# nv-tlabs/NKSR

Hardware: AMD Instinct MI355X
Metric: reconstructed points/sec (solve+mesh) (higher is better)
Workload: dtype f32

## Files before the change

### include/nksr_hip.h

```cpp
#ifndef NKSR_HIP_H
#define NKSR_HIP_H
#include <stddef.h>
#include <stdint.h>

#ifdef __cplusplus
extern "C" {
#endif

#define NKSR_MAX_DEPTH 6
#define NKSR_OK 0
#define NKSR_ERR_ARG (-1)
#define NKSR_ERR_HIP (-2)
#define NKSR_ERR_CAPACITY (-3)

const char* nksr_last_error(void);
int nksr_version(void);

typedef struct {
    int32_t n;
    int32_t offset;
    const int64_t* keys;
    const int32_t* ijk;
    const int32_t* nbr;
    const int64_t* hkeys;
// ... 98 lines not shown
    const int32_t* row_index;
    int64_t level_base;
} nksr_siteset_t;

int nksr_assemble_count(const nksr_hier_t* h, void* workspace, int32_t* rowcount, int32_t* crosscount, int32_t* samelow,
                        int32_t* indeg, void* stream);
size_t nksr_assemble_workspace_bytes(const nksr_hier_t* h);
size_t nksr_assemble_split_bytes(const nksr_hier_t* h, int64_t total_rows);
int nksr_assemble(const nksr_hier_t* h, const nksr_siteset_t* sets, int nsets, float reg, int col_bits,
                  void* workspace, const int32_t* rowptr, const int32_t* indeg, const int32_t* samelow,
                  const int32_t* mir_off, int col_format, int32_t* cols_out, float* vals_out, float* diag_out,
                  uint64_t* mir_keys, float* mir_vals, float* b_out, void* split_scratch, size_t split_scratch_bytes, void* stream);
int nksr_place_mirrors(const uint64_t* keys_sorted, const float* vals_sorted, int64_t n, int col_bits,
                       const int32_t* rowptr, const int32_t* mirptr, int col_format, int32_t* cols_out, float* vals_out,
                       void* stream);

size_t nksr_spmv_workspace_bytes(int64_t nnz);
int nksr_spmv_plan(const int32_t* rowptr, int32_t M, int64_t nnz, int col_format, void* workspace, void* stream);
int nksr_spmv_csr(const int32_t* rowptr, const void* cols, const float* vals, int32_t M, int64_t nnz, int col_format,
                  const float* x, float* y, void* workspace, void* stream);
int nksr_pack_cols21(const int32_t* cols32, int64_t n_padded, uint64_t* packed_out, void* stream);
int nksr_spmv_set_variant(int v);
size_t nksr_pcg_workspace_bytes(int32_t M, int64_t nnz);
struct nksr_coarse_precond_s;
int nksr_pcg_solve(const int32_t* rowptr, const void* cols, const float* vals, const float* diag, int32_t M,
                   int64_t nnz, int col_format, const float* b, float* x, float tol, int max_iter, int check_every,
                   void* workspace, const struct nksr_coarse_precond_s* coarse_precond, double* info_out, void* stream);
int nksr_pcg_profile(int enable, double* ms_out, int64_t* launches_out);
int64_t nksr_pcg_profile_samples(float* ms_out, int64_t capacity);
int nksr_pcg_profile_bytes(double* algorithmic_out, double* physical_out);
// ... 283 lines not shown
```

### nksr_amd/csrc/assemble.hip

```cpp
#include "common.h"
#include <stdlib.h>

#define ASM_WAVES 1

struct AsmArgs {
    nksr_hier_t hier;
    nksr_siteset_t sets[3];
    int nsets;
    int M;
    int col_bits;
    float reg;
    float* blocks[NKSR_MAX_DEPTH];
    float* bvec[NKSR_MAX_DEPTH];
    int32_t* nsites[NKSR_MAX_DEPTH];
    int32_t* colmap[NKSR_MAX_DEPTH];
    int col_format;
};

__device__ __forceinline__ int row_level(const nksr_hier_t& h, int row) {
    int d = 0;
    while (d + 1 < h.depth && row >= h.lv[d + 1].offset) ++d;
    return d;
}

// ... 7 lines not shown
    const uint32_t t = kk / 192u, m = kk - t * 192u;
    return (int64_t)(t * 192u + 3u * (m & 63u) + (m >> 6));
}

typedef float asm_f32x16 __attribute__((ext_vector_type(16)));

__device__ __forceinline__ float asm_row_value(const nksr_siteset_t& S, int64_t q, int L, int d, int col) {
    if (!S.level_stride) return S.val[(q * L + d) * 27 + col];
    const int dd = col / 27, s = col - dd * 27;
    const int64_t site = S.ncomp == 1 ? q : q / 3;
    const int64_t row = (S.row_index ? (int64_t)S.row_index[site] : site * S.ncomp) + (q - site * S.ncomp);
    return S.val[((int64_t)(d + dd - S.level_base) * S.level_stride + row) * 27 + s];
}

template <int NT>
__device__ __forceinline__ void cell_blocks_finalize(const AsmArgs& A, int d, int c, int lane, asm_f32x16 (&acc)[NT], int total) {
    const nksr_level_t& lv = A.hier.lv[d];
    const int T = (A.hier.depth - d) * 27;
    const int j = lane & 31, half = lane >> 5;
    if (lane == 0) A.nsites[d][c] = total;
    if (total == 0) return;
    float* out = A.blocks[d] + (int64_t)c * 27 * T;
    float* bv = A.bvec[d] + (int64_t)c * 27;
    const int nb = (lane < 27) ? lv.nbr[(int64_t)c * 27 + lane] : -1;
    const unsigned long long need = __ballot(nb >= 0);
#pragma unroll
    for (int n = 0; n < NT; ++n) {
        const int col = 32 * n + j;
#pragma unroll
        for (int r = 0; r < 16; ++r) {
            const int s = (r & 3) + 8 * (r >> 2) + 4 * half;
            if (s < 27 && ((need >> s) & 1ull)) {
                if (col < T) out[s * T + col] = acc[n][r];
                else if (col == T) bv[s] = acc[n][r];
            }
        }
    }
}

#define ASM_PART_ROWS 128
#define ASM_TRIP 4
__host__ __device__ __forceinline__ int asm_level_parts(int d) {
    const int k = d >= 2 ? (1 << (2 * (d - 2))) : 1;
    return k > 64 ? 64 : k;
}
__device__ __forceinline__ int asm_cell_rows(const AsmArgs& A, int d, int c) {
    int R = 0;
    for (int si = 0; si < A.nsets; ++si) R += (A.sets[si].end[d][c] - A.sets[si].start[d][c]) * A.sets[si].ncomp;
    return R;
// ... 27 lines not shown
__device__ __forceinline__ void asm_lm_mfma(const AsmLanePtr<NT>& P, int r0, int r_hi, int half, int j, float w, float (&b)[ASM_TRIP][NT], asm_f32x16 (&acc)[NT]) {
#pragma unroll
    for (int u = 0; u < ASM_TRIP; ++u) {
        const bool ok = r0 + 2 * u + half < r_hi;
        float v[NT];
#pragma unroll
        for (int n = 0; n < NT; ++n) v[n] = (ok && P.on[n]) ? b[u][n] : 0.f;
        const float a = (j < 27) ? w * v[0] : 0.f;
#pragma unroll
        for (int n = 0; n < NT; ++n) acc[n] = __builtin_amdgcn_mfma_f32_32x32x2f32(a, v[n], acc[n], 0, 0, 0);
    }
}
template <int NT>
__device__ __forceinline__ void asm_lm_pointers(const AsmArgs& A, int d, int lane, AsmLanePtr<NT>& P) {
    const nksr_siteset_t& S = A.sets[0];
    const int L = A.hier.depth;
    const int T = (L - d) * 27;
    const int j = lane & 31;
#pragma unroll
    for (int n = 0; n < NT; ++n) {
        const int col = 32 * n + j;
        const int dd = col / 27, sl = col - dd * 27;
        P.on[n] = col < T || (col == T && S.target);
        P.mul[n] = (col == T && S.target) ? 1 : 27;
        P.p[n] = (col == T && S.target) ? S.target : S.val + (col < T ? (int64_t)(d + dd - S.level_base) * S.level_stride * 27 + sl : (int64_t)(d - S.level_base) * S.level_stride * 27);
    }
}
template <int NT>
__device__ __forceinline__ void asm_accumulate_lm(const AsmArgs& A, int d, int r_lo, int r_hi, int lane, asm_f32x16 (&acc)[NT]) {
    if (r_hi <= r_lo) return;
    const nksr_siteset_t& S = A.sets[0];
    const int j = lane & 31, half = lane >> 5;
    AsmLanePtr<NT> P;
    asm_lm_pointers<NT>(A, d, lane, P);
    const float w = S.weight;
    float bA[ASM_TRIP][NT], bB[ASM_TRIP][NT];
    asm_lm_load<NT>(P, r_lo, r_lo, r_hi, half, bA);
    for (int r0 = r_lo; r0 < r_hi; r0 += 4 * ASM_TRIP) {
        const int r1 = r0 + 2 * ASM_TRIP, r2 = r0 + 4 * ASM_TRIP;
        if (r1 < r_hi) asm_lm_load<NT>(P, r1, r_lo, r_hi, half, bB);
// ... 75 lines not shown
    if (c >= A.hier.lv[d].n) return;
    asm_f32x16 acc[NT];
#pragma unroll
    for (int n = 0; n < NT; ++n)
#pragma unroll
        for (int r = 0; r < 16; ++r) acc[n][r] = 0.f;
    for (int p = 0; p < nsplit; ++p) {
        const float* in = scratch + ((int64_t)c * nsplit + p) * (NT * 16 * 64) + lane;
#pragma unroll
        for (int n = 0; n < NT; ++n)
#pragma unroll
            for (int r = 0; r < 16; ++r) acc[n][r] += in[(n * 16 + r) * 64];
    }
    int total = 0;
    for (int si = 0; si < A.nsets; ++si) total += A.sets[si].end[d][c] - A.sets[si].start[d][c];
    cell_blocks_finalize<NT>(A, d, c, lane, acc, total);
}

template <int NT>
__global__ void __launch_bounds__(ASM_WAVES * 64) k_cell_blocks_seq(AsmArgs A, int d, int nsplit) {
    const int wave = threadIdx.x >> 6, lane = threadIdx.x & 63;
    const int c = blockIdx.x * ASM_WAVES + wave;
    if (c >= A.hier.lv[d].n) return;
    asm_f32x16 tot[NT];
#pragma unroll
    for (int n = 0; n < NT; ++n)
#pragma unroll
        for (int r = 0; r < 16; ++r) tot[n][r] = 0.f;
    const int R = asm_cell_rows(A, d, c);
    for (int p = 0; p < nsplit; ++p) {
        int lo, hi;
// ... 2 lines not shown
#pragma unroll
        for (int n = 0; n < NT; ++n)
#pragma unroll
            for (int r = 0; r < 16; ++r) acc[n][r] = 0.f;
        if (hi > lo) {
            if (asm_is_row_list(A)) asm_accumulate_lm<NT>(A, d, A.sets[0].start[d][c] + lo, A.sets[0].start[d][c] + hi, lane, acc);
            else asm_accumulate_rows<NT>(A, d, c, lo, hi, lane, acc);
        }
#pragma unroll
        for (int n = 0; n < NT; ++n)
#pragma unroll
            for (int r = 0; r < 16; ++r) tot[n][r] += acc[n][r];
    }
    int total = 0;
    for (int si = 0; si < A.nsets; ++si) total += A.sets[si].end[d][c] - A.sets[si].start[d][c];
    cell_blocks_finalize<NT>(A, d, c, lane, tot, total);
}

template <int NT, bool LM>
__global__ void __launch_bounds__(ASM_WAVES * 64) k_cell_blocks(AsmArgs A, int d) {
    const int wave = threadIdx.x >> 6, lane = threadIdx.x & 63;
    const nksr_level_t& lv = A.hier.lv[d];
    const int c = blockIdx.x * ASM_WAVES + wave;
    if (c >= lv.n) return;
    const int L = A.hier.depth;
    const int T = (L - d) * 27;
    const int j = lane & 31, half = lane >> 5;
    asm_f32x16 acc[NT];
#pragma unroll
    for (int n = 0; n < NT; ++n)
#pragma unroll
        for (int r = 0; r < 16; ++r) acc[n][r] = 0.f;
    int total = 0;
    if (LM && asm_is_row_list(A)) {
        const int k0 = A.sets[0].start[d][c], k1 = A.sets[0].end[d][c];
        total = k1 > k0 ? k1 - k0 : 0;
        asm_accumulate_lm<NT>(A, d, k0, k1, lane, acc);
        cell_blocks_finalize<NT>(A, d, c, lane, acc, total);
        return;
    }
    for (int si = 0; si < A.nsets; ++si) {
        const nksr_siteset_t& S = A.sets[si];
        const int k0 = S.start[d][c], k1 = S.end[d][c];
        if (k0 >= k1) continue;
        total += k1 - k0;
        const int64_t q0 = (int64_t)k0 * S.ncomp;
        const int nrows = (k1 - k0) * S.ncomp;
        const float w = S.weight;
        if (!LM) {
            for (int m0 = 0; m0 < nrows; m0 += 2) {
                const bool valid = m0 + half < nrows;
                const int64_t q = q0 + m0 + half;
                const float* ra = S.val + (q * L + d) * 27;
// ... 143 lines not shown

template <int NQ> struct cols_u { float v[NQ]; } __attribute__((packed, aligned(4)));
template <int NQ>
__device__ __forceinline__ void load_cols(const float* __restrict__ row, int lane, int T, float out[NQ]) {
    const int t0 = NQ * lane;
    if (t0 + NQ <= T) {
        const cols_u<NQ> c = *reinterpret_cast<const cols_u<NQ>*>(row + t0);
#pragma unroll
        for (int q = 0; q < NQ; ++q) out[q] = c.v[q];
    } else {
#pragma unroll
        for (int q = 0; q < NQ; ++q) out[q] = (t0 + q < T) ? row[t0 + q] : 0.f;
    }
}

template <int NQ>
__global__ void __launch_bounds__(ASM_WAVES * 64) k_row_fill(AsmArgs A, const int32_t* __restrict__ rowptr,
                                                             const int32_t* __restrict__ indeg, const int32_t* __restrict__ samelow,
                                                             const int32_t* __restrict__ mir_off,
                                                             int32_t* __restrict__ cols_out, float* __restrict__ vals_out,
                                                             float* __restrict__ diag_out, uint64_t* __restrict__ mir_keys,
                                                             float* __restrict__ mir_vals,
                                                             float* __restrict__ b_out, int row_begin, int row_end) {
    extern __shared__ __attribute__((aligned(16))) float lds[];
    const int wave = threadIdx.x >> 6, lane = threadIdx.x & 63;
    const int row = row_begin + blockIdx.x * ASM_WAVES + wave;
    if (row >= row_end) return;
    const nksr_hier_t& h = A.hier;
    const int L = h.depth;
    const int d = row_level(h, row);
    const nksr_level_t& lv = h.lv[d];
    const int i = row - lv.offset;
    const int ix = lv.ijk[i * 3], iy = lv.ijk[i * 3 + 1], iz = lv.ijk[i * 3 + 2];
    const int nslots = (L - d) * 125;
    const int T = (L - d) * 27;
    float* acc = lds + wave * (NKSR_MAX_DEPTH * 125);
    for (int t = lane; t < nslots; t += 64) acc[t] = 0.f;

    const int cme = (lane < 27) ? lv.nbr[(int64_t)i * 27 + lane] : -1;
    const int nse = (cme >= 0) ? A.nsites[d][cme] : 0;
    unsigned long long act = __ballot(nse > 0);
    float bl = (nse > 0) ? A.bvec[d][(int64_t)cme * 27 + (26 - lane)] : 0.f;
#pragma unroll
    for (int o = 32; o > 0; o >>= 1) bl += __shfl_xor(bl, o);
    if (lane == 0) b_out[row] = bl;

    int edd[NQ], esx[NQ], esy[NQ], esz[NQ];
#pragma unroll
    for (int q = 0; q < NQ; ++q) {
        const int t = NQ * lane + q, s = t % 27;
        edd[q] = t / 27;
        esx[q] = s / 9 - 1; esy[q] = (s / 3) % 3 - 1; esz[q] = s % 3 - 1;
    }
    constexpr int RF_BATCH = 4;
    float vb[2][RF_BATCH][NQ];
    int sp[2][RF_BATCH];
    auto fetch = [&](int buf) {
#pragma unroll
        for (int u = 0; u < RF_BATCH; ++u) {
            sp[buf][u] = -1;
// ... 21 lines not shown
                    acc[dd * 125 + (rz * 5 + ry) * 5 + rx] += vb[buf][u][q];
                }
            }
        }
    };
    fetch(0);
    while (sp[0][0] >= 0) {
        fetch(1);
        accumulate(0);
        if (sp[1][0] < 0) break;
        fetch(0);
        accumulate(1);
    }

    const int32_t* cm = A.colmap[d] + (int64_t)i * nslots;
    int64_t lpos = (int64_t)rowptr[row] + indeg[row];
    int64_t opos = lpos + samelow[row];
    int64_t mpos = (int64_t)mir_off[row];
    for (int t0 = 0; t0 < nslots; t0 += 64) {
        const int t = t0 + lane;
        const int cv = (t < nslots) ? cm[t] : -1;
        const bool up = cv >= 0, low = cv <= -2, mir = up && t >= 125;
        const unsigned long long mu = __ballot(up), ml = __ballot(low), mm = __ballot(mir);
        const unsigned long long below = (1ull << lane) - 1ull;
        if (up | low) {
            const float v = acc[t];
            const int64_t k = up ? opos + __popcll(mu & below) : lpos + __popcll(ml & below);
            const int64_t ph = csr_phys(k, A.col_format);
            cols_out[ph] = up ? cv : -2 - cv;
            vals_out[ph] = v;
// ... 17 lines not shown
}

__global__ void k_place_mirrors(const uint64_t* __restrict__ keys, const float* __restrict__ vals, int64_t n, int col_bits,
                                const int32_t* __restrict__ rowptr, const int32_t* __restrict__ mirptr,
                                int32_t* __restrict__ cols_out, float* __restrict__ vals_out, int fmt) {
    int64_t m = (int64_t)blockIdx.x * blockDim.x + threadIdx.x;
    if (m >= n) return;
    const uint64_t key = keys[m];
    const int r = (int)(key & (((uint64_t)1 << col_bits) - 1));
    const int src = (int)(key >> col_bits);
    const int64_t ph = csr_phys((int64_t)rowptr[r] + (m - (int64_t)mirptr[r]), fmt);
    cols_out[ph] = src;
    vals_out[ph] = vals[m];
}

static int fill_args(AsmArgs& A, const nksr_hier_t* h, const nksr_siteset_t* sets, int nsets, float reg, int col_bits,
                     void* workspace) {
    if (h->depth < 1 || h->depth > NKSR_MAX_DEPTH) return nksr_set_error(NKSR_ERR_ARG, "bad depth %d", h->depth);
    if (nsets < 0 || nsets > 3) return nksr_set_error(NKSR_ERR_ARG, "at most 3 site sets");
    memset(&A, 0, sizeof(A));
    A.hier = *h;
    for (int s = 0; s < nsets; ++s) {
        if (!(sets[s].weight >= 0.f)) return nksr_set_error(NKSR_ERR_ARG, "site-set weights must be >= 0 (set %d: %g)", s, (double)sets[s].weight);
        A.sets[s] = sets[s];
    }
    A.nsets = nsets;
    A.M = h->lv[h->depth - 1].offset + h->lv[h->depth - 1].n;
    A.col_bits = col_bits;
    A.reg = reg;
    if (col_bits < 1 || col_bits > 32 || ((int64_t)1 << col_bits) < A.M) return nksr_set_error(NKSR_ERR_ARG, "col_bits too small");
// ... 36 lines not shown
extern "C" int nksr_assemble_count(const nksr_hier_t* h, void* workspace, int32_t* rowcount, int32_t* crosscount, int32_t* samelow,
                                   int32_t* indeg, void* stream) {
    AsmArgs A;
    int M = h->lv[h->depth - 1].offset + h->lv[h->depth - 1].n;
    int cb = 1;
    while (((int64_t)1 << cb) < M) ++cb;
    int rc = fill_args(A, h, nullptr, 0, 0.f, cb, workspace);
    if (rc) return rc;
    if (A.M <= 0) return NKSR_OK;
    hipLaunchKernelGGL(k_row_count, dim3(nksr_blocks(A.M, ASM_WAVES * RC_RUN)), dim3(ASM_WAVES * 64), 0, (hipStream_t)stream, A, rowcount,
                       crosscount, samelow, indeg);
    NKSR_CHECK_LAUNCH();
    return NKSR_OK;
}

extern "C" int nksr_assemble(const nksr_hier_t* h, const nksr_siteset_t* sets, int nsets, float reg, int col_bits,
                             void* workspace, const int32_t* rowptr, const int32_t* indeg, const int32_t* samelow,
                             const int32_t* mir_off, int col_format,
                             int32_t* cols_out, float* vals_out, float* diag_out, uint64_t* mir_keys, float* mir_vals,
                             float* b_out, void* split_scratch, size_t split_scratch_bytes, void* stream) {
    AsmArgs A;
    int rc = fill_args(A, h, sets, nsets, reg, col_bits, workspace);
    if (rc) return rc;
    if (col_format < 0 || col_format > 2) return nksr_set_error(NKSR_ERR_ARG, "col_format must be 0, 1 or 2");
    A.col_format = col_format;
    if (A.M <= 0) return NKSR_OK;
    hipStream_t st = (hipStream_t)stream;
    const dim3 blk(ASM_WAVES * 64);
    const size_t lds = (size_t)ASM_WAVES * NKSR_MAX_DEPTH * 125 * sizeof(float);
    int64_t total_rows = 0;
    bool lm = false;
    for (int si = 0; si < nsets; ++si) {
        total_rows += sets[si].n * sets[si].ncomp;
        if (si > 0 && (sets[si].level_stride != 0) != lm) return nksr_set_error(NKSR_ERR_ARG, "site sets mix site-major and level-major rows");
        if (sets[si].level_base < 0 || sets[si].level_base >= h->depth || (sets[si].level_base > 0 && !sets[si].level_stride))
            return nksr_set_error(NKSR_ERR_ARG, "site set: level_base needs level-major rows and a level of the hierarchy");
        lm = sets[si].level_stride != 0;
        for (int d = 0; d < sets[si].level_base; ++d)
            if (h->lv[d].n > 0) return nksr_set_error(NKSR_ERR_ARG, "site set: rows start at level %d but level %d of the hierarchy has cells", (int)sets[si].level_base, d);
    }
    for (int d = 0; d < h->depth; ++d) {
        const int n = h->lv[d].n;
        if (n <= 0) continue;
        const int T = (h->depth - d) * 27, NT = (T + 32) / 32;
// ... 14 lines not shown
                case 5: CELLSPLIT(5); break;
                default: CELLSPLIT(6); break;
            }
        } else {
            switch (NT) {
                case 1: if (lm) hipLaunchKernelGGL((k_cell_blocks<1, true>), grid, blk, 0, st, A, d); else hipLaunchKernelGGL((k_cell_blocks<1, false>), grid, blk, 0, st, A, d); break;
                case 2: if (lm) hipLaunchKernelGGL((k_cell_blocks<2, true>), grid, blk, 0, st, A, d); else hipLaunchKernelGGL((k_cell_blocks<2, false>), grid, blk, 0, st, A, d); break;
                case 3: if (lm) hipLaunchKernelGGL((k_cell_blocks<3, true>), grid, blk, 0, st, A, d); else hipLaunchKernelGGL((k_cell_blocks<3, false>), grid, blk, 0, st, A, d); break;
                case 4: if (lm) hipLaunchKernelGGL((k_cell_blocks<4, true>), grid, blk, 0, st, A, d); else hipLaunchKernelGGL((k_cell_blocks<4, false>), grid, blk, 0, st, A, d); break;
                case 5: if (lm) hipLaunchKernelGGL((k_cell_blocks<5, true>), grid, blk, 0, st, A, d); else hipLaunchKernelGGL((k_cell_blocks<5, false>), grid, blk, 0, st, A, d); break;
                default: if (lm) hipLaunchKernelGGL((k_cell_blocks<6, true>), grid, blk, 0, st, A, d); else hipLaunchKernelGGL((k_cell_blocks<6, false>), grid, blk, 0, st, A, d); break;
            }
        }
        NKSR_CHECK_LAUNCH();
    }
    for (int d = 0; d < h->depth; ++d) {
        const int n = h->lv[d].n;
        if (n <= 0) continue;
        const int T = (h->depth - d) * 27;
        const int r0 = h->lv[d].offset, r1 = r0 + n;
        const dim3 grid(nksr_blocks(n, ASM_WAVES));
#define ROWFILL(NQ) hipLaunchKernelGGL((k_row_fill<NQ>), grid, blk, lds, st, A, rowptr, indeg, samelow, mir_off, cols_out, vals_out, diag_out, \
                                       mir_keys, mir_vals, b_out, r0, r1)
        if (T > 128) ROWFILL(3); else if (T > 64) ROWFILL(2); else ROWFILL(1);
        NKSR_CHECK_LAUNCH();
    }
    return NKSR_OK;
}

extern "C" int nksr_place_mirrors(const uint64_t* keys_sorted, const float* vals_sorted, int64_t n, int col_bits,
                                  const int32_t* rowptr, const int32_t* mirptr, int col_format, int32_t* cols_out, float* vals_out,
                                  void* stream) {
    if (n <= 0) return NKSR_OK;
    if (col_format < 0 || col_format > 2) return nksr_set_error(NKSR_ERR_ARG, "col_format must be 0, 1 or 2");
    hipLaunchKernelGGL(k_place_mirrors, dim3(nksr_blocks(n, 256)), dim3(256), 0, (hipStream_t)stream, keys_sorted, vals_sorted, n,
                       col_bits, rowptr, mirptr, cols_out, vals_out, col_format);
    NKSR_CHECK_LAUNCH();
    return NKSR_OK;
}
```

### nksr_amd/fields/assembly.py

```python
import ctypes as C
import time

import torch

from .. import _lib, ops
from .._lib import SiteSetT, call, ptr, stream
from ._timing import _tick


def _sets_from_operator(fld, fused_op, coarse_from, sets, keep):
    first, last = fused_op['span'][0], fused_op['span'][1]
    st_all, en_all = first.clamp(min=0), (last + 1).contiguous()
    off = fld.svh.offsets
    S = sets[0]
    S.n, S.ncomp, S.weight = fused_op['rows_total'], 1, 1.0
    if fused_op.get('row_format') == 'factors':
        dense = fld._dense_coarse_rows(fused_op, int(coarse_from))
        S.val, S.level_base = ptr(dense), int(coarse_from)
        keep.append(dense)
    else:
        S.val = ptr(fused_op['rows_all'])
    S.level_stride = fused_op['rows_total']
    for d in range(fld.svh.depth):
        nd = fld.svh.level(d).num_voxels
# ... 74 lines not shown
    del ws
    ks, vs = ops.sort_pairs(mir_k, mir_v.view(torch.int32), end_bit=col_bits)
    del mir_k, mir_v
    call('nksr_place_mirrors', ptr(ks), ptr(vs.view(torch.float32)), n_mir, col_bits, ptr(rowptr), ptr(mirptr), fmt, ptr(cols),
         ptr(vals), stream())
    del ks, vs
    td = _tick('asm:mirrors', td)
    if fmt == 1:
        packed = torch.empty(npad // 3, dtype=torch.int64, device=dev)
        call('nksr_pack_cols21', ptr(cols), npad, ptr(packed), stream())
        cols = packed
    if coarse_from is None:
        fld.nnz = nnz
    del keep
    return rowptr, cols, vals, diag, b
```

### nksr_amd/fields/coarse_precond.py

```python
import ctypes as C
import os
import time

import torch

from .. import ops
from .._lib import PC_MAX_STEPS, CoarsePrecondT, call, ptr, stream
from ._timing import _tick

PC_RATIO = 40.0
PC_DROP_TOL = 0.005


def _pack_block(rowptr, cols, vals, diag, n, row_seg, counts, drop):
    dev = rowptr.device
    ar = torch.arange(n, dtype=torch.int64, device=dev)
    old_of_new = torch.argsort(row_seg.long() * n + ar)
    new_of_old = torch.empty_like(old_of_new)
    new_of_old[old_of_new] = ar
    seg_base = torch.cat([counts.new_zeros(1), torch.cumsum(counts, 0)]).to(torch.int32)
    row_seg_new = row_seg[old_of_new].contiguous()
    o2n, n2o = old_of_new.to(torch.int32), new_of_old.to(torch.int32)
    lens = torch.empty(n + 1, dtype=torch.int32, device=dev)
    lens[n:] = 0
    call('nksr_coarse_pack_count', ptr(rowptr), ptr(cols), ptr(vals), ptr(diag), n, ptr(o2n), drop, ptr(lens), stream())
    prow = ops.exclusive_sum_i32(lens)
    kept = int(prow[n].item())
    packed = torch.empty(max(kept, 1), dtype=torch.int32, device=dev)
    dis = torch.empty(n, dtype=torch.float32, device=dev)
    call('nksr_coarse_pack', ptr(rowptr), ptr(cols), ptr(vals), ptr(diag), n, ptr(o2n), ptr(n2o), ptr(row_seg_new), ptr(seg_base), ptr(prow),
         drop, ptr(packed), ptr(dis), stream())
    return packed, prow, dis, o2n, seg_base, row_seg_new, kept


def coarse_precond(fld, op, reg_weight, segments=None, sites=None, override=None):
    cfg = fld.solver_config.get('coarse_precond')
    L = fld.svh.depth
    if cfg is False:
        return None
    cfg = dict(cfg) if isinstance(cfg, dict) else dict(override or {})
    for k, e in (('first_level', 'NKSR_PC_LEVEL'), ('steps', 'NKSR_PC_STEPS'), ('ratio', 'NKSR_PC_RATIO')):
        if e in os.environ and k not in cfg:
            cfg[k] = float(os.environ[e])
    c0 = int(cfg.get('first_level', 2))
    off = fld.svh.offsets
    M = fld.svh.num_unknowns
    if not 0 < c0 < L or M - off[c0] < 1:
        return None
    n = M - off[c0]
    nseg = segments.nseg if segments is not None else 1
    td = _tick('_', time.perf_counter())
    if op is not None:
        rowptr, cols, vals, diag, _ = fld.assemble(None, None, None, 1.0, 1.0, reg_weight, coarse_from=c0, fused_op=op)
    else:
        rowptr, cols, vals, diag, _ = fld.assemble(reg_weight=reg_weight, coarse_from=c0, **sites)
    td = _tick('pc:assemble', td)
    lam = torch.empty(nseg, dtype=torch.float32, device=fld.device)
    coef = torch.empty(nseg * (1 + 2 * PC_MAX_STEPS), dtype=torch.float32, device=fld.device)
    row_seg = segments.unknown_seg[off[c0]:].contiguous() if segments is not None else None
    pc = CoarsePrecondT()
    pc.first, pc.n, pc.steps, pc.lambda_scale, pc.ratio = off[c0], n, int(cfg.get('steps', 8)), float(cfg.get('lambda_scale', 1.1)), float(cfg.get('ratio', PC_RATIO))
    gersh = torch.empty(nseg, dtype=torch.float32, device=fld.device)
    pc.lambda_, pc.coef = ptr(lam), ptr(coef)
    nnz = int(cols.numel())
    info = {'first_level': c0, 'unknowns': n, 'nnz': nnz, 'steps': int(pc.steps), 'lambda': lam}
    rs = row_seg if row_seg is not None else torch.zeros(n, dtype=torch.int32, device=fld.device)
    counts = torch.bincount(rs.long(), minlength=nseg)
    if cfg.get('packed', os.environ.get('NKSR_PC_PACKED', '1') != '0') and int(counts.max()) < 65536:
        drop = float(cfg.get('drop', os.environ.get('NKSR_PC_DROP', PC_DROP_TOL)))
        packed, prow, dis, o2n, seg_base, row_seg_new, kept = _pack_block(rowptr, cols, vals, diag, n, rs, counts, drop)
        info.update(nnz_kept=kept + n, drop=drop)
        work = torch.empty(4 * n, dtype=torch.float32, device=fld.device)
        if 'steps' not in cfg and (segments is not None or n >= 100000):
            pc.steps = 10
            info['steps'] = 10
        pc.format, pc.row_seg, pc.work = 1, ptr(row_seg_new), ptr(work)
        pc.packed, pc.packed_rowptr, pc.dis, pc.old_of_new, pc.seg_base = ptr(packed), ptr(prow), ptr(dis), ptr(o2n), ptr(seg_base)
        call('nksr_coarse_lambda_max_packed', C.byref(pc), nseg, 8, ptr(work), ptr(lam), stream())
        call('nksr_coarse_gershgorin', C.byref(pc), nseg, ptr(work), ptr(gersh), stream())
        pc.gersh = ptr(gersh)
        info.update(packed=True, gershgorin=gersh, keep=(packed, prow, dis, o2n, seg_base, row_seg_new, work, lam, coef, gersh))
        td = _tick('pc:pack+lambda', td)
        return dict(info, pc=pc)
    work = torch.empty(3 * n, dtype=torch.float32, device=fld.device)
    call('nksr_coarse_lambda_max', ptr(rowptr), ptr(cols), ptr(vals), ptr(diag), n, 8, ptr(work), ptr(lam),
# ... 8 lines not shown
```

### nksr_amd/ops.py

```python
import threading

import torch

from ._lib import call, ptr, stream, with_tmp


def _bits(n):
    b = 1
    while (1 << b) < max(int(n), 1):
        b += 1
    return b


class KeyBits:

    def __init__(self, lo, hi, depth=1):
        self.lo, self.hi = [int(v) for v in lo], [int(v) for v in hi]
        self.reach = 2 << max(int(depth) - 1, 0)

    def bits(self, level=0):
        b = 0
        for a in range(3):
            bias = 1 << (20 - level)
            lo = ((self.lo[a] - self.reach) >> level) - 2 + bias
# ... 16 lines not shown
        return self.kb

    def __exit__(self, *exc):
        _tls.hint = self.prev


def varying_bits(keys, level=None):
    hint = getattr(_tls, 'hint', None)
    if level is not None and hint is not None:
        return hint.bits(level)
    if keys.numel() < (1 << 17):
        return 63
    return max(1, int((keys ^ keys[:1]).max()).bit_length())


def sort_keys(keys, end_bit=None, level=None):
    n = keys.numel()
    out = torch.empty_like(keys)
    if n:
        if end_bit is None:
            end_bit = varying_bits(keys, level)
        with_tmp('nksr_sort_keys_u64', keys.device, ptr(keys), ptr(out), n, 0, int(end_bit), stream())
    return out


def sort_pairs(keys, vals32, end_bit=None, pad=0, level=None):
    n = keys.numel()
    ko = torch.empty_like(keys)
    vo = torch.zeros(n + pad, dtype=vals32.dtype, device=vals32.device)[:n] if pad else torch.empty_like(vals32)
    if n:
        if end_bit is None:
            end_bit = varying_bits(keys, level)
        with_tmp('nksr_sort_pairs_u64_u32', keys.device, ptr(keys), ptr(ko), ptr(vals32), ptr(vo), n, 0, int(end_bit), stream())
    return ko, vo


def unique_sorted(keys_sorted):
# ... 89 lines not shown
```

Before: 31.08 million.

## Assemble coarse preconditioner directly into packed half-precision format

Adds a packed assembly path that builds the coarse preconditioner matrix straight from the cell blocks. Rows are renumbered per segment, values are scaled by the inverse square-root diagonal, stored as fp16 and small entries dropped, all inside the row-fill kernel. This replaces the earlier route of assembling a full CSR and then running a separate pack pass, so the intermediate matrix materialisation and its extra passes go away. In exchange it adds new kernels (diagonal, mirror compaction, run and length computation, row packing), a partial key sort, and extra host syncs through .item() calls. It also changes the lane-to-column mapping in the LM block accumulation to a per-level layout.

```diff
diff --git a/include/nksr_hip.h b/include/nksr_hip.h
--- a/include/nksr_hip.h
+++ b/include/nksr_hip.h
@@ -136,6 +136,17 @@
 int nksr_place_mirrors(const uint64_t* keys_sorted, const float* vals_sorted, int64_t n, int col_bits,
                        const int32_t* rowptr, const int32_t* mirptr, int col_format, int32_t* cols_out, float* vals_out,
                        void* stream);
+int nksr_assemble_packed(const nksr_hier_t* h, const nksr_siteset_t* sets, int nsets, float reg, void* workspace,
+                         const int32_t* samelow, const int32_t* mir_off, const int32_t* own_off, const int32_t* new_of_old,
+                         const int32_t* local_col, float drop_tol, float* diag_out, uint32_t* own_out, uint64_t* mir_out,
+                         int32_t* kept_out, void* split_scratch, size_t split_scratch_bytes, void* stream);
+int nksr_packed_mirrors_compact(int32_t n, const uint64_t* mir_staged, const int32_t* mir_off, const int32_t* kept_mir,
+                                const int32_t* kept_off, uint64_t* mir_dense, void* stream);
+int nksr_packed_row_lengths(int32_t n, const uint64_t* mir_sorted, int64_t n_mir, const int32_t* kept, const int32_t* old_of_new,
+                            int32_t* runs_out, int32_t* lens_out, void* stream);
+int nksr_packed_rows(int32_t n, const uint64_t* mir_sorted, const int32_t* runs, const uint32_t* own, const int32_t* own_off,
+                     const int32_t* samelow, const int32_t* kept, const int32_t* old_of_new, const int32_t* packed_rowptr,
+                     const float* diag, uint32_t* packed_out, float* dis_out, void* stream);
 
 size_t nksr_spmv_workspace_bytes(int64_t nnz);
 int nksr_spmv_plan(const int32_t* rowptr, int32_t M, int64_t nnz, int col_format, void* workspace, void* stream);
diff --git a/nksr_amd/csrc/assemble.hip b/nksr_amd/csrc/assemble.hip
--- a/nksr_amd/csrc/assemble.hip
+++ b/nksr_amd/csrc/assemble.hip
@@ -1,5 +1,6 @@
 #include "common.h"
 #include <stdlib.h>
+#include <hip/hip_fp16.h>
 
 #define ASM_WAVES 1
 
@@ -45,7 +46,7 @@
 }
 
 template <int NT>
-__device__ __forceinline__ void cell_blocks_finalize(const AsmArgs& A, int d, int c, int lane, asm_f32x16 (&acc)[NT], int total) {
+__device__ __forceinline__ void cell_blocks_finalize(const AsmArgs& A, int d, int c, int lane, asm_f32x16 (&acc)[NT], int total, bool by_level = false) {
     const nksr_level_t& lv = A.hier.lv[d];
     const int T = (A.hier.depth - d) * 27;
     const int j = lane & 31, half = lane >> 5;
@@ -62,8 +63,13 @@
         for (int r = 0; r < 16; ++r) {
             const int s = (r & 3) + 8 * (r >> 2) + 4 * half;
             if (s < 27 && ((need >> s) & 1ull)) {
-                if (col < T) out[s * T + col] = acc[n][r];
-                else if (col == T) bv[s] = acc[n][r];
+                if (by_level) {
+                    if (j < 27) { if (27 * n < T) out[s * T + 27 * n + j] = acc[n][r]; }
+                    else if (n == 0 && j == 27) bv[s] = acc[n][r];
+                } else {
+                    if (col < T) out[s * T + col] = acc[n][r];
+                    else if (col == T) bv[s] = acc[n][r];
+                }
             }
         }
     }
@@ -121,16 +127,15 @@
 template <int NT>
 __device__ __forceinline__ void asm_lm_pointers(const AsmArgs& A, int d, int lane, AsmLanePtr<NT>& P) {
     const nksr_siteset_t& S = A.sets[0];
-    const int L = A.hier.depth;
-    const int T = (L - d) * 27;
+    const int levels = A.hier.depth - d;
     const int j = lane & 31;
 #pragma unroll
     for (int n = 0; n < NT; ++n) {
-        const int col = 32 * n + j;
-        const int dd = col / 27, sl = col - dd * 27;
-        P.on[n] = col < T || (col == T && S.target);
-        P.mul[n] = (col == T && S.target) ? 1 : 27;
-        P.p[n] = (col == T && S.target) ? S.target : S.val + (col < T ? (int64_t)(d + dd - S.level_base) * S.level_stride * 27 + sl : (int64_t)(d - S.level_base) * S.level_stride * 27);
+        const bool rhs = n == 0 && j == 27 && S.target;
+        const int dd = n < levels ? n : 0;
+        P.on[n] = (n < levels && j < 27) || rhs;
+        P.mul[n] = rhs ? 1 : 27;
+        P.p[n] = rhs ? S.target : S.val + (int64_t)(d + dd - S.level_base) * S.level_stride * 27 + (j < 27 ? j : 26);
     }
 }
 template <int NT>
@@ -236,7 +241,7 @@
     }
     int total = 0;
     for (int si = 0; si < A.nsets; ++si) total += A.sets[si].end[d][c] - A.sets[si].start[d][c];
-    cell_blocks_finalize<NT>(A, d, c, lane, acc, total);
+    cell_blocks_finalize<NT>(A, d, c, lane, acc, total, asm_is_row_list(A));
 }
 
 template <int NT>
@@ -269,7 +274,7 @@
     }
     int total = 0;
     for (int si = 0; si < A.nsets; ++si) total += A.sets[si].end[d][c] - A.sets[si].start[d][c];
-    cell_blocks_finalize<NT>(A, d, c, lane, tot, total);
+    cell_blocks_finalize<NT>(A, d, c, lane, tot, total, asm_is_row_list(A));
 }
 
 template <int NT, bool LM>
@@ -291,7 +296,7 @@
         const int k0 = A.sets[0].start[d][c], k1 = A.sets[0].end[d][c];
         total = k1 > k0 ? k1 - k0 : 0;
         asm_accumulate_lm<NT>(A, d, k0, k1, lane, acc);
-        cell_blocks_finalize<NT>(A, d, c, lane, acc, total);
+        cell_blocks_finalize<NT>(A, d, c, lane, acc, total, true);
         return;
     }
     for (int si = 0; si < A.nsets; ++si) {
@@ -465,14 +470,47 @@
     }
 }
 
-template <int NQ>
+__device__ __forceinline__ __half cc_scaled(float v, float di, float dj) { return __float2half_rn(v * (di * dj)); }
+__device__ __forceinline__ bool cc_keep(__half hv, float drop) { return fabsf(__half2float(hv)) >= drop; }
+
+struct AsmPackOut {
+    const float* diag;
+    const int32_t* new_of_old;
+    const int32_t* local;
+    const int32_t* own_off;
+    uint32_t* own;
+    uint64_t* mir;
+    int32_t* kept;
+    float drop;
+};
+
+__global__ void __launch_bounds__(256) k_row_diag(AsmArgs A, float* __restrict__ diag) {
+    const int row = (blockIdx.x * 256 + threadIdx.x) >> 5, l = threadIdx.x & 31;
+    if (row >= A.M) return;
+    const nksr_hier_t& h = A.hier;
+    const int d = row_level(h, row);
+    const nksr_level_t& lv = h.lv[d];
+    const int i = row - lv.offset;
+    const int T = (h.depth - d) * 27;
+    const int c = (l < 27) ? lv.nbr[(int64_t)i * 27 + l] : -1;
+    const int on = (c >= 0 && A.nsites[d][c] > 0) ? 1 : 0;
+    const float x = on ? A.blocks[d][((int64_t)c * 27 + (26 - l)) * T + (26 - l)] : 0.f;
+    float s = 0.f;
+    for (int sp = 0; sp < 27; ++sp) {
+        const float v = __shfl(x, sp, 32);
+        if (__shfl(on, sp, 32)) s += v;
+    }
+    if (l == 0) diag[row] = s + A.reg;
+}
+
+template <int NQ, bool PACK>
 __global__ void __launch_bounds__(ASM_WAVES * 64) k_row_fill(AsmArgs A, const int32_t* __restrict__ rowptr,
                                                              const int32_t* __restrict__ indeg, const int32_t* __restrict__ samelow,
                                                              const int32_t* __restrict__ mir_off,
                                                              int32_t* __restrict__ cols_out, float* __restrict__ vals_out,
                                                              float* __restrict__ diag_out, uint64_t* __restrict__ mir_keys,
                                                              float* __restrict__ mir_vals,
-                                                             float* __restrict__ b_out, int row_begin, int row_end) {
+                                                             float* __restrict__ b_out, int row_begin, int row_end, AsmPackOut K) {
     extern __shared__ __attribute__((aligned(16))) float lds[];
     const int wave = threadIdx.x >> 6, lane = threadIdx.x & 63;
     const int row = row_begin + blockIdx.x * ASM_WAVES + wave;
@@ -491,10 +529,12 @@
     const int cme = (lane < 27) ? lv.nbr[(int64_t)i * 27 + lane] : -1;
     const int nse = (cme >= 0) ? A.nsites[d][cme] : 0;
     unsigned long long act = __ballot(nse > 0);
-    float bl = (nse > 0) ? A.bvec[d][(int64_t)cme * 27 + (26 - lane)] : 0.f;
-#pragma unroll
-    for (int o = 32; o > 0; o >>= 1) bl += __shfl_xor(bl, o);
-    if (lane == 0) b_out[row] = bl;
+    if (!PACK) {
+        float bl = (nse > 0) ? A.bvec[d][(int64_t)cme * 27 + (26 - lane)] : 0.f;
+#pragma unroll
+        for (int o = 32; o > 0; o >>= 1) bl += __shfl_xor(bl, o);
+        if (lane == 0) b_out[row] = bl;
+    }
 
     int edd[NQ], esx[NQ], esy[NQ], esz[NQ];
 #pragma unroll
@@ -546,6 +586,46 @@
     }
 
     const int32_t* cm = A.colmap[d] + (int64_t)i * nslots;
+    if (PACK) {
+        const float di = 1.f / sqrtf(K.diag[row]);
+        const int local = K.local[row];
+        const int base = K.new_of_old[row] - local;
+        int lpos = K.own_off[row];
+        int opos = lpos + samelow[row];
+        int mpos = mir_off[row];
+        const int l0 = lpos, o0 = opos, m0 = mpos;
+        for (int t0 = 0; t0 < nslots; t0 += 64) {
+            const int t = t0 + lane;
+            const int cv = (t < nslots) ? cm[t] : -1;
+            const bool up = cv >= 0, low = cv <= -2;
+            bool keep = false;
+            uint32_t hbits = 0u;
+            int ncol = 0;
+            if (up | low) {
+                const int col = up ? cv : -2 - cv;
+                const __half hv = cc_scaled(acc[t], di, 1.f / sqrtf(K.diag[col]));
+                keep = cc_keep(hv, K.drop);
+                hbits = (uint32_t)__half_as_ushort(hv) << 16;
+                ncol = K.new_of_old[col];
+            }
+            const bool ku = keep && up, kl = keep && low, km = ku && t >= 125;
+            const unsigned long long mu = __ballot(ku), ml = __ballot(kl), mm = __ballot(km);
+            const unsigned long long below = (1ull << lane) - 1ull;
+            if (keep) {
+                K.own[ku ? opos + __popcll(mu & below) : lpos + __popcll(ml & below)] = hbits | (uint32_t)(ncol - base);
+                if (km) K.mir[mpos + __popcll(mm & below)] = ((uint64_t)(uint32_t)ncol << 32) | (uint64_t)(hbits | ((uint32_t)local & 0xFFFFu));
+            }
+            opos += __popcll(mu);
+            lpos += __popcll(ml);
+            mpos += __popcll(mm);
+        }
+        if (lane == 0) {
+            K.kept[row] = lpos - l0;
+            K.kept[(int64_t)(A.M + 1) + row] = opos - o0;
+            K.kept[2 * (int64_t)(A.M + 1) + row] = mpos - m0;
+        }
+        return;
+    }
     int64_t lpos = (int64_t)rowptr[row] + indeg[row];
     int64_t opos = lpos + samelow[row];
     int64_t mpos = (int64_t)mir_off[row];
@@ -593,6 +673,51 @@
     vals_out[ph] = vals[m];
 }
 
+__global__ void __launch_bounds__(256) k_pk_compact(int M, const uint64_t* __restrict__ staged, const int32_t* __restrict__ mir_off,
+                                                    const int32_t* __restrict__ kept, const int32_t* __restrict__ kept_off,
+                                                    uint64_t* __restrict__ dense) {
+    const int r = (blockIdx.x * 256 + threadIdx.x) >> 4, l = threadIdx.x & 15;
+    if (r >= M) return;
+    const int n = kept[r], src = mir_off[r], dst = kept_off[r];
+    for (int k = l; k < n; k += 16) dense[dst + k] = staged[src + k];
+}
+
+__global__ void __launch_bounds__(256) k_pk_runs(const uint64_t* __restrict__ sorted, int nk, int n, int32_t* __restrict__ runs) {
+    const int m = blockIdx.x * 256 + threadIdx.x;
+    if (m >= nk) return;
+    const int d = (int)(sorted[m] >> 32);
+    if (m == 0 || (int)(sorted[m - 1] >> 32) != d) runs[d] = m;
+    if (m == nk - 1 || (int)(sorted[m + 1] >> 32) != d) runs[n + d] = m + 1;
+}
+
+__global__ void __launch_bounds__(256) k_pk_lens(int n, const int32_t* __restrict__ runs, const int32_t* __restrict__ kept,
+                                                 const int32_t* __restrict__ old_of_new, int32_t* __restrict__ lens) {
+    const int i = blockIdx.x * 256 + threadIdx.x;
+    if (i >= n) return;
+    const int o = old_of_new[i];
+    lens[i] = (runs[n + i] - runs[i]) + kept[o] + kept[(int64_t)(n + 1) + o];
+}
+
+__global__ void __launch_bounds__(256) k_pk_rows(int n, const uint64_t* __restrict__ sorted, const int32_t* __restrict__ runs,
+                                                 const uint32_t* __restrict__ own, const int32_t* __restrict__ own_off,
+                                                 const int32_t* __restrict__ samelow, const int32_t* __restrict__ kept,
+                                                 const int32_t* __restrict__ old_of_new, const int32_t* __restrict__ prow,
+                                                 const float* __restrict__ diag, uint32_t* __restrict__ pk, float* __restrict__ dis) {
+    const int i = (blockIdx.x * 256 + threadIdx.x) >> 4, l = threadIdx.x & 15;
+    if (i >= n) return;
+    const int o = old_of_new[i];
+    int p = prow[i];
+    const int mb = runs[i], nm = runs[n + i] - mb;
+    for (int k = l; k < nm; k += 16) pk[p + k] = (uint32_t)sorted[mb + k];
+    p += nm;
+    const int lo = own_off[o], nl = kept[o], nu = kept[(int64_t)(n + 1) + o];
+    for (int k = l; k < nl; k += 16) pk[p + k] = own[lo + k];
+    p += nl;
+    const int up = lo + samelow[o];
+    for (int k = l; k < nu; k += 16) pk[p + k] = own[up + k];
+    if (l == 0) dis[i] = 1.f / sqrtf(diag[o]);
+}
+
 static int fill_args(AsmArgs& A, const nksr_hier_t* h, const nksr_siteset_t* sets, int nsets, float reg, int col_bits,
                      void* workspace) {
     if (h->depth < 1 || h->depth > NKSR_MAX_DEPTH) return nksr_set_error(NKSR_ERR_ARG, "bad depth %d", h->depth);
@@ -659,20 +784,9 @@
     return NKSR_OK;
 }
 
-extern "C" int nksr_assemble(const nksr_hier_t* h, const nksr_siteset_t* sets, int nsets, float reg, int col_bits,
-                             void* workspace, const int32_t* rowptr, const int32_t* indeg, const int32_t* samelow,
-                             const int32_t* mir_off, int col_format,
-                             int32_t* cols_out, float* vals_out, float* diag_out, uint64_t* mir_keys, float* mir_vals,
-                             float* b_out, void* split_scratch, size_t split_scratch_bytes, void* stream) {
-    AsmArgs A;
-    int rc = fill_args(A, h, sets, nsets, reg, col_bits, workspace);
-    if (rc) return rc;
-    if (col_format < 0 || col_format > 2) return nksr_set_error(NKSR_ERR_ARG, "col_format must be 0, 1 or 2");
-    A.col_format = col_format;
-    if (A.M <= 0) return NKSR_OK;
-    hipStream_t st = (hipStream_t)stream;
+static int launch_cell_blocks(const AsmArgs& A, const nksr_hier_t* h, const nksr_siteset_t* sets, int nsets, void* split_scratch,
+                              size_t split_scratch_bytes, hipStream_t st) {
     const dim3 blk(ASM_WAVES * 64);
-    const size_t lds = (size_t)ASM_WAVES * NKSR_MAX_DEPTH * 125 * sizeof(float);
     int64_t total_rows = 0;
     bool lm = false;
     for (int si = 0; si < nsets; ++si) {
@@ -717,17 +831,104 @@
         }
         NKSR_CHECK_LAUNCH();
     }
+    return NKSR_OK;
+}
+
+static int launch_row_fill(const AsmArgs& A, const nksr_hier_t* h, const int32_t* rowptr, const int32_t* indeg, const int32_t* samelow,
+                           const int32_t* mir_off, int32_t* cols_out, float* vals_out, float* diag_out, uint64_t* mir_keys,
+                           float* mir_vals, float* b_out, const AsmPackOut* K, hipStream_t st) {
+    const dim3 blk(ASM_WAVES * 64);
+    const size_t lds = (size_t)ASM_WAVES * NKSR_MAX_DEPTH * 125 * sizeof(float);
+    AsmPackOut none;
+    memset(&none, 0, sizeof(none));
     for (int d = 0; d < h->depth; ++d) {
         const int n = h->lv[d].n;
         if (n <= 0) continue;
         const int T = (h->depth - d) * 27;
         const int r0 = h->lv[d].offset, r1 = r0 + n;
         const dim3 grid(nksr_blocks(n, ASM_WAVES));
-#define ROWFILL(NQ) hipLaunchKernelGGL((k_row_fill<NQ>), grid, blk, lds, st, A, rowptr, indeg, samelow, mir_off, cols_out, vals_out, diag_out, \
-                                       mir_keys, mir_vals, b_out, r0, r1)
+#define ROWFILL(NQ) do { if (K) hipLaunchKernelGGL((k_row_fill<NQ, true>), grid, blk, lds, st, A, rowptr, indeg, samelow, mir_off, cols_out, vals_out, \
+                                                   diag_out, mir_keys, mir_vals, b_out, r0, r1, *K); \
+                         else hipLaunchKernelGGL((k_row_fill<NQ, false>), grid, blk, lds, st, A, rowptr, indeg, samelow, mir_off, cols_out, vals_out, \
+                                                 diag_out, mir_keys, mir_vals, b_out, r0, r1, none); } while (0)
         if (T > 128) ROWFILL(3); else if (T > 64) ROWFILL(2); else ROWFILL(1);
         NKSR_CHECK_LAUNCH();
     }
+    return NKSR_OK;
+}
+
+extern "C" int nksr_assemble(const nksr_hier_t* h, const nksr_siteset_t* sets, int nsets, float reg, int col_bits,
+                             void* workspace, const int32_t* rowptr, const int32_t* indeg, const int32_t* samelow,
+                             const int32_t* mir_off, int col_format,
+                             int32_t* cols_out, float* vals_out, float* diag_out, uint64_t* mir_keys, float* mir_vals,
+                             float* b_out, void* split_scratch, size_t split_scratch_bytes, void* stream) {
+    AsmArgs A;
+    int rc = fill_args(A, h, sets, nsets, reg, col_bits, workspace);
+    if (rc) return rc;
+    if (col_format < 0 || col_format > 2) return nksr_set_error(NKSR_ERR_ARG, "col_format must be 0, 1 or 2");
+    A.col_format = col_format;
+    if (A.M <= 0) return NKSR_OK;
+    rc = launch_cell_blocks(A, h, sets, nsets, split_scratch, split_scratch_bytes, (hipStream_t)stream);
+    if (rc) return rc;
+    return launch_row_fill(A, h, rowptr, indeg, samelow, mir_off, cols_out, vals_out, diag_out, mir_keys, mir_vals, b_out, nullptr,
+                           (hipStream_t)stream);
+}
+
+extern "C" int nksr_assemble_packed(const nksr_hier_t* h, const nksr_siteset_t* sets, int nsets, float reg, void* workspace,
+                                    const int32_t* samelow, const int32_t* mir_off, const int32_t* own_off, const int32_t* new_of_old,
+                                    const int32_t* local_col, float drop_tol, float* diag_out, uint32_t* own_out, uint64_t* mir_out,
+                                    int32_t* kept_out, void* split_scratch, size_t split_scratch_bytes, void* stream) {
+    AsmArgs A;
+    int rc = fill_args(A, h, sets, nsets, reg, 32, workspace);
+    if (rc) return rc;
+    if (!samelow || !mir_off || !own_off || !new_of_old || !local_col || !diag_out || !own_out || !mir_out || !kept_out)
+        return nksr_set_error(NKSR_ERR_ARG, "NULL arrays");
+    if (!(drop_tol >= 0.f) || drop_tol >= 1.f) return nksr_set_error(NKSR_ERR_ARG, "drop_tol must be in [0, 1)");
+    A.col_format = 2;
+    if (A.M <= 0) return NKSR_OK;
+    hipStream_t st = (hipStream_t)stream;
+    rc = launch_cell_blocks(A, h, sets, nsets, split_scratch, split_scratch_bytes, st);
+    if (rc) return rc;
+    hipLaunchKernelGGL(k_row_diag, dim3(nksr_blocks((int64_t)A.M * 32, 256)), dim3(256), 0, st, A, diag_out);
+    NKSR_CHECK_LAUNCH();
+    AsmPackOut K;
+    K.diag = diag_out; K.new_of_old = new_of_old; K.local = local_col; K.own_off = own_off;
+    K.own = own_out; K.mir = mir_out; K.kept = kept_out; K.drop = drop_tol;
+    return launch_row_fill(A, h, nullptr, nullptr, samelow, mir_off, nullptr, nullptr, nullptr, nullptr, nullptr, nullptr, &K, st);
+}
+
+extern "C" int nksr_packed_mirrors_compact(int32_t n, const uint64_t* mir_staged, const int32_t* mir_off, const int32_t* kept_mir,
+                                           const int32_t* kept_off, uint64_t* mir_dense, void* stream) {
+    if (n <= 0) return NKSR_OK;
+    if (!mir_staged || !mir_off || !kept_mir || !kept_off || !mir_dense) return nksr_set_error(NKSR_ERR_ARG, "NULL arrays");
+    hipLaunchKernelGGL(k_pk_compact, dim3(nksr_blocks((int64_t)n * 16, 256)), dim3(256), 0, (hipStream_t)stream, n, mir_staged, mir_off,
+                       kept_mir, kept_off, mir_dense);
+    NKSR_CHECK_LAUNCH();
+    return NKSR_OK;
+}
+
+extern "C" int nksr_packed_row_lengths(int32_t n, const uint64_t* mir_sorted, int64_t n_mir, const int32_t* kept, const int32_t* old_of_new,
+                                       int32_t* runs_out, int32_t* lens_out, void* stream) {
+    if (n <= 0) return NKSR_OK;
+    if ((n_mir > 0 && !mir_sorted) || !kept || !old_of_new || !runs_out || !lens_out) return nksr_set_error(NKSR_ERR_ARG, "NULL arrays");
+    if (n_mir < 0 || n_mir >= ((int64_t)1 << 31)) return nksr_set_error(NKSR_ERR_ARG, "bad mirror count");
+    hipStream_t st = (hipStream_t)stream;
+    NKSR_CHECK_HIP(hipMemsetAsync(runs_out, 0, 2 * (size_t)n * sizeof(int32_t), st));
+    if (n_mir > 0) hipLaunchKernelGGL(k_pk_runs, dim3(nksr_blocks(n_mir, 256)), dim3(256), 0, st, mir_sorted, (int)n_mir, n, runs_out);
+    hipLaunchKernelGGL(k_pk_lens, dim3(nksr_blocks(n, 256)), dim3(256), 0, st, n, (const int32_t*)runs_out, kept, old_of_new, lens_out);
+    NKSR_CHECK_LAUNCH();
+    return NKSR_OK;
+}
+
+extern "C" int nksr_packed_rows(int32_t n, const uint64_t* mir_sorted, const int32_t* runs, const uint32_t* own, const int32_t* own_off,
+                                const int32_t* samelow, const int32_t* kept, const int32_t* old_of_new, const int32_t* packed_rowptr,
+                                const float* diag, uint32_t* packed_out, float* dis_out, void* stream) {
+    if (n <= 0) return NKSR_OK;
+    if (!runs || !own || !own_off || !samelow || !kept || !old_of_new || !packed_rowptr || !diag || !packed_out || !dis_out)
+        return nksr_set_error(NKSR_ERR_ARG, "NULL arrays");
+    hipLaunchKernelGGL(k_pk_rows, dim3(nksr_blocks((int64_t)n * 16, 256)), dim3(256), 0, (hipStream_t)stream, n, mir_sorted, runs, own, own_off,
+                       samelow, kept, old_of_new, packed_rowptr, diag, packed_out, dis_out);
+    NKSR_CHECK_LAUNCH();
     return NKSR_OK;
 }
 
diff --git a/nksr_amd/fields/assembly.py b/nksr_amd/fields/assembly.py
--- a/nksr_amd/fields/assembly.py
+++ b/nksr_amd/fields/assembly.py
@@ -112,3 +112,58 @@
         fld.nnz = nnz
     del keep
     return rowptr, cols, vals, diag, b
+
+
+def assemble_packed(fld, reg_weight, coarse_from, fused_op, old_of_new, new_of_old, local_col, drop):
+    dev = fld.device
+    c0 = int(coarse_from)
+    hier = fld._coarse_hier(c0)
+    M = fld.svh.num_unknowns - fld.svh.offsets[c0]
+    if M == 0:
+        raise RuntimeError('empty hierarchy')
+    keep = []
+    sets = (SiteSetT * 2)()
+    nsets = _sets_from_operator(fld, fused_op, c0, sets, keep)
+    counts = torch.zeros((4, M + 1), dtype=torch.int32, device=dev)
+    rowcount, crosscount, samelow, indeg = counts[0], counts[1], counts[2], counts[3]
+    ws = torch.empty(int(_lib.lib.nksr_assemble_workspace_bytes(C.byref(hier))), dtype=torch.uint8, device=dev)
+    td = _tick('_', time.perf_counter())
+    call('nksr_assemble_count', C.byref(hier), ptr(ws), ptr(rowcount), ptr(crosscount), ptr(samelow), ptr(indeg), stream())
+    n_up, n_mir = [int(v) for v in counts[:2].sum(dim=1, dtype=torch.int64).tolist()]
+    td = _tick('asm:count', td)
+    nnz = 2 * n_up + M
+    if nnz >= 2 ** 31 - 4096:
+        raise RuntimeError('coarse block too large (M=%d, nnz=%d >= 2^31)' % (M, nnz))
+    own_off = ops.exclusive_sum_i32(samelow + rowcount)
+    mir_off = ops.exclusive_sum_i32(crosscount)
+    own = torch.empty(max(2 * n_up - n_mir, 1), dtype=torch.int32, device=dev)
+    mir = torch.empty(max(n_mir, 1), dtype=torch.int64, device=dev)
+    kept = torch.empty((3, M + 1), dtype=torch.int32, device=dev)
+    kept[:, M] = 0
+    diag = torch.empty(M, dtype=torch.float32, device=dev)
+    split_bytes = int(_lib.lib.nksr_assemble_split_bytes(C.byref(hier), sum(int(sets[i].n) * int(sets[i].ncomp) for i in range(nsets))))
+    split = torch.empty(split_bytes, dtype=torch.uint8, device=dev) if split_bytes else None
+    call('nksr_assemble_packed', C.byref(hier), sets, nsets, float(reg_weight), ptr(ws), ptr(samelow), ptr(mir_off), ptr(own_off),
+         ptr(new_of_old), ptr(local_col), float(drop), ptr(diag), ptr(own), ptr(mir), ptr(kept), ptr(split), split_bytes, stream())
+    td = _tick('asm:blocks+fill', td)
+    del split, ws, keep
+    kept_off = ops.exclusive_sum_i32(kept[2])
+    n_kept_mir = int(kept_off[M].item())
+    dense = torch.empty(n_kept_mir, dtype=torch.int64, device=dev)
+    if n_kept_mir:
+        call('nksr_packed_mirrors_compact', M, ptr(mir), ptr(mir_off), ptr(kept[2]), ptr(kept_off), ptr(dense), stream())
+    del mir
+    srt = ops.sort_keys(dense, begin_bit=32, end_bit=32 + ops._bits(M))
+    del dense
+    runs = torch.empty(2 * M, dtype=torch.int32, device=dev)
+    lens = torch.empty(M + 1, dtype=torch.int32, device=dev)
+    lens[M:] = 0
+    call('nksr_packed_row_lengths', M, ptr(srt), n_kept_mir, ptr(kept), ptr(old_of_new), ptr(runs), ptr(lens), stream())
+    prow = ops.exclusive_sum_i32(lens)
+    n_kept = int(prow[M].item())
+    packed = torch.empty(max(n_kept, 1), dtype=torch.int32, device=dev)
+    dis = torch.empty(M, dtype=torch.float32, device=dev)
+    call('nksr_packed_rows', M, ptr(srt), ptr(runs), ptr(own), ptr(own_off), ptr(samelow), ptr(kept), ptr(old_of_new), ptr(prow),
+         ptr(diag), ptr(packed), ptr(dis), stream())
+    td = _tick('asm:mirrors+pack', td)
+    return packed, prow, dis, n_kept, nnz, diag
diff --git a/nksr_amd/fields/coarse_precond.py b/nksr_amd/fields/coarse_precond.py
--- a/nksr_amd/fields/coarse_precond.py
+++ b/nksr_amd/fields/coarse_precond.py
@@ -5,6 +5,7 @@
 import torch
 
 from .. import ops
+from . import assembly
 from .._lib import PC_MAX_STEPS, CoarsePrecondT, call, ptr, stream
 from ._timing import _tick
 
@@ -12,15 +13,18 @@
 PC_DROP_TOL = 0.005
 
 
-def _pack_block(rowptr, cols, vals, diag, n, row_seg, counts, drop):
-    dev = rowptr.device
-    ar = torch.arange(n, dtype=torch.int64, device=dev)
+def _renumber(n, row_seg, counts):
+    ar = torch.arange(n, dtype=torch.int64, device=row_seg.device)
     old_of_new = torch.argsort(row_seg.long() * n + ar)
     new_of_old = torch.empty_like(old_of_new)
     new_of_old[old_of_new] = ar
     seg_base = torch.cat([counts.new_zeros(1), torch.cumsum(counts, 0)]).to(torch.int32)
-    row_seg_new = row_seg[old_of_new].contiguous()
-    o2n, n2o = old_of_new.to(torch.int32), new_of_old.to(torch.int32)
+    return old_of_new.to(torch.int32), new_of_old.to(torch.int32), seg_base, row_seg[old_of_new].contiguous()
+
+
+def _pack_block(rowptr, cols, vals, diag, n, row_seg, counts, drop):
+    dev = rowptr.device
+    o2n, n2o, seg_base, row_seg_new = _renumber(n, row_seg, counts)
     lens = torch.empty(n + 1, dtype=torch.int32, device=dev)
     lens[n:] = 0
     call('nksr_coarse_pack_count', ptr(rowptr), ptr(cols), ptr(vals), ptr(diag), n, ptr(o2n), drop, ptr(lens), stream())
@@ -50,25 +54,33 @@
     n = M - off[c0]
     nseg = segments.nseg if segments is not None else 1
     td = _tick('_', time.perf_counter())
-    if op is not None:
+    row_seg = segments.unknown_seg[off[c0]:].contiguous() if segments is not None else None
+    rs = row_seg if row_seg is not None else torch.zeros(n, dtype=torch.int32, device=fld.device)
+    counts = torch.bincount(rs.long(), minlength=nseg)
+    pack = bool(cfg.get('packed', os.environ.get('NKSR_PC_PACKED', '1') != '0')) and int(counts.max()) < 65536
+    drop = float(cfg.get('drop', os.environ.get('NKSR_PC_DROP', PC_DROP_TOL)))
+    direct = pack and op is not None and bool(cfg.get('direct', True))
+    if direct:
+        o2n, n2o, seg_base, row_seg_new = _renumber(n, rs, counts)
+        local = (n2o - seg_base[rs.long()]).contiguous()
+        packed, prow, dis, kept, nnz, _ = assembly.assemble_packed(fld, reg_weight, c0, op, o2n, n2o, local, drop)
+    elif op is not None:
         rowptr, cols, vals, diag, _ = fld.assemble(None, None, None, 1.0, 1.0, reg_weight, coarse_from=c0, fused_op=op)
     else:
         rowptr, cols, vals, diag, _ = fld.assemble(reg_weight=reg_weight, coarse_from=c0, **sites)
     td = _tick('pc:assemble', td)
     lam = torch.empty(nseg, dtype=torch.float32, device=fld.device)
     coef = torch.empty(nseg * (1 + 2 * PC_MAX_STEPS), dtype=torch.float32, device=fld.device)
-    row_seg = segments.unknown_seg[off[c0]:].contiguous() if segments is not None else None
     pc = CoarsePrecondT()
     pc.first, pc.n, pc.steps, pc.lambda_scale, pc.ratio = off[c0], n, int(cfg.get('steps', 8)), float(cfg.get('lambda_scale', 1.1)), float(cfg.get('ratio', PC_RATIO))
     gersh = torch.empty(nseg, dtype=torch.float32, device=fld.device)
     pc.lambda_, pc.coef = ptr(lam), ptr(coef)
-    nnz = int(cols.numel())
+    if not direct:
+        nnz = int(cols.numel())
     info = {'first_level': c0, 'unknowns': n, 'nnz': nnz, 'steps': int(pc.steps), 'lambda': lam}
-    rs = row_seg if row_seg is not None else torch.zeros(n, dtype=torch.int32, device=fld.device)
-    counts = torch.bincount(rs.long(), minlength=nseg)
-    if cfg.get('packed', os.environ.get('NKSR_PC_PACKED', '1') != '0') and int(counts.max()) < 65536:
-        drop = float(cfg.get('drop', os.environ.get('NKSR_PC_DROP', PC_DROP_TOL)))
-        packed, prow, dis, o2n, seg_base, row_seg_new, kept = _pack_block(rowptr, cols, vals, diag, n, rs, counts, drop)
+    if pack:
+        if not direct:
+            packed, prow, dis, o2n, seg_base, row_seg_new, kept = _pack_block(rowptr, cols, vals, diag, n, rs, counts, drop)
         info.update(nnz_kept=kept + n, drop=drop)
         work = torch.empty(4 * n, dtype=torch.float32, device=fld.device)
         if 'steps' not in cfg and (segments is not None or n >= 100000):
diff --git a/nksr_amd/ops.py b/nksr_amd/ops.py
--- a/nksr_amd/ops.py
+++ b/nksr_amd/ops.py
@@ -54,13 +54,13 @@
     return max(1, int((keys ^ keys[:1]).max()).bit_length())
 
 
-def sort_keys(keys, end_bit=None, level=None):
+def sort_keys(keys, end_bit=None, level=None, begin_bit=0):
     n = keys.numel()
     out = torch.empty_like(keys)
     if n:
         if end_bit is None:
             end_bit = varying_bits(keys, level)
-        with_tmp('nksr_sort_keys_u64', keys.device, ptr(keys), ptr(out), n, 0, int(end_bit), stream())
+        with_tmp('nksr_sort_keys_u64', keys.device, ptr(keys), ptr(out), n, int(begin_bit), int(end_bit), stream())
     return out
 
 
```

After: 31.68 million (median of 6 runs). 1.02x the previous value.
